# ddlau/modular_rl

Measured on AMD Instinct MI355X. Metric: env-steps/sec + TRPO-iters/sec, 4096 envs×1024 steps, 1/2/4/8 MI355X, higher is better.
Workload: dtype fp32

## Files before the change

### modular_rl_amd/csrc/fvp_split_role.h

```cpp
#pragma once
#include "../../include/mrl_hip.h"
#include "bf16_frag.h"
#include "mlp_device.h"
#include "rows_epilogue.h"

namespace mrl {

__host__ __device__ constexpr int split_fw(const BDims& b) { return b.fwd_words - b.fa0; }
__host__ __device__ constexpr int split_fwd_words(const BDims& b) { return b.fa0 + 3 * split_fw(b); }

__device__ inline float bf16_part(float v, int p) {
  const __bf16 a = (__bf16)v;
  if (p == 0) return (float)a;
  const float r = v - (float)a;
  const __bf16 c = (__bf16)r;
  if (p == 1) return (float)c;
  return r - (float)c;
}

__device__ inline int split_image_items(const BDims& b) { return b.fa0 + split_fw(b); }

__device__ inline void split_image_item(const MlpDims& d, const BDims& b, const float* th, float* image, int u) {
  if (u < b.fa0) {
    int idx;
    if (u < b.fb1) idx = d.fb0 + (u - b.fb0);
    else if (u < b.hv) idx = d.fb1 + (u - b.fb1);
    else if (u < b.hb) idx = d.hv + (u - b.hv);
    else idx = d.hb + (u - b.hb);
    image[u] = image_value(d, th, idx);
    return;
  }
  const int FW = split_fw(b);
  const int wp = u;
  int seg, rel;
  if (wp < b.fa1) { seg = 0; rel = wp - b.fa0; }
  else { seg = 1; rel = wp - b.fa1; }
  const int frag = rel >> 2, q = rel & 3;
  const float lo = bimage_elem(d, b, th, seg, frag, 2 * q), hi = bimage_elem(d, b, th, seg, frag, 2 * q + 1);
#pragma unroll
  for (int part = 0; part < 3; ++part) {
    const __bf16 l = (__bf16)bf16_part(lo, part), h = (__bf16)bf16_part(hi, part);
    image[u + part * FW] =
        __uint_as_float((uint32_t)__builtin_bit_cast(uint16_t, l) | ((uint32_t)__builtin_bit_cast(uint16_t, h) << 16));
  }
}

__device__ inline void split8v(const float* v, bf16x8* out) {
#pragma unroll
  for (int j = 0; j < 8; j += 2) {
    bf16x2 a, c, e;
    split2(f32x2{v[j], v[j + 1]}, a, c, e);
    out[0][j] = a[0];
    out[0][j + 1] = a[1];
    out[1][j] = c[0];
    out[1][j + 1] = c[1];
    out[2][j] = e[0];
    out[2][j + 1] = e[1];
  }
}
__device__ inline void split8(const f32x16& t, int sp, bf16x8* out) {
  float v[8];
#pragma unroll
  for (int j = 0; j < 8; ++j) v[j] = t[8 * sp + j];
  split8v(v, out);
}

__device__ inline void mfma_split(const float* img, int seg, int PS, int f, int lane, const bf16x8* x, f32x16& acc) {
  const bf16x8 w0 = frag_at(img, seg, f, lane), w1 = frag_at(img, seg + PS, f, lane);
  const bf16x8 w2 = frag_at(img, seg + 2 * PS, f, lane);
  acc = MFMA32B(w2, x[0], acc);
  acc = MFMA32B(w0, x[2], acc);
  acc = MFMA32B(w1, x[1], acc);
  acc = MFMA32B(w1, x[0], acc);
  acc = MFMA32B(w0, x[1], acc);
  acc = MFMA32B(w0, x[0], acc);
}

#define FVP_SPLIT_FENCE() __builtin_amdgcn_sched_barrier(0)

template <int SH>
__device__ inline void split_shape(RowsArgs& a, BDims& b) {
  if constexpr (SH != 0) {
    constexpr StaticShape S = STATIC_SHAPES[SH];
    a.d = static_dims(SH);
    a.A = S.A;
    a.head = S.head;
    a.n_obs = S.O;
    a.gh = S.head == MRL_HEAD_GAUSS ? 2 * S.A : S.A;
    a.ept = nullptr;
    b = bf16_dims(S.O, S.A);
  }
}

struct JvpSplitRole {
  RowsArgs a;
  BDims b;
  const float* img;
  const float* imt;
  MlpDims dd;
  int lane, h, PS;
  bool need_z;
  float xv[MAX_KS0B][8];
  f32x16 h1[2];

  __device__ __forceinline__ void init(const RowsArgs& a_, const BDims& b_, const float* img_, const float* imt_,
                                       int lane_) {
    a = a_;
    b = b_;
    img = img_;
    imt = imt_;
    dd = head_dims(a.d, b);
    lane = lane_;
    h = lane >> 5;
    PS = split_fw(b);
    need_z = a.head != MRL_HEAD_GAUSS;
  }
  __device__ __forceinline__ void load_xh1(int64_t t, float (&x)[MAX_KS0B][8], f32x16* hh) {
    const int64_t r = t * 32 + (lane & 31);
    XGlobalNB xl{a.x, a.ept, a.ts_limit, a.n_obs, r, r < a.n};
#pragma unroll
    for (int s0 = 0; s0 < MAX_KS0B; ++s0)
#pragma unroll
      for (int j = 0; j < 8; ++j) x[s0][j] = s0 < b.KS0B ? xl(16 * s0 + 8 * h + j) : 0.f;
    cache_load(a.cache + t * CACHE_TILE_FLOATS, lane, 0, hh[0]);
    cache_load(a.cache + t * CACHE_TILE_FLOATS, lane, 1, hh[1]);
  }
  __device__ __forceinline__ void prologue(int64_t tile) { load_xh1(tile, xv, h1); }
  template <bool PF = true, class Sink>
  __device__ __forceinline__ void tile(int64_t tile, int64_t tn, Sink&& sink) {
    const int64_t row = tile * 32 + (lane & 31);
    const bool valid = row < a.n;
    const float* ct = a.cache + tile * CACHE_TILE_FLOATS;
    f32x16 h2[2];
    if constexpr (PF) {
      cache_load(ct, lane, 2, h2[0]);
      cache_load(ct, lane, 3, h2[1]);
      __builtin_amdgcn_sched_barrier(0);
    }
    float xn[MAX_KS0B][8];
    f32x16 h1n[2];
    if constexpr (PF) load_xh1(tn, xn, h1n);
    else load_xh1(tile, xv, h1);
    __builtin_amdgcn_sched_barrier(0);
    f32x16 dh[2];
    dh[0] = load_bias16(imt, b.fb0, 0, h);
    dh[1] = load_bias16(imt, b.fb0, 1, h);
#pragma unroll
    for (int s0 = 0; s0 < MAX_KS0B; ++s0) {
      if (s0 < b.KS0B) {
        bf16x8 xs[3];
        split8v(xv[s0], xs);
        mfma_split(imt, b.fa0, PS, 0 * b.KS0B + s0, lane, xs, dh[0]);
        mfma_split(imt, b.fa0, PS, 1 * b.KS0B + s0, lane, xs, dh[1]);
      }
    }
    mul_dtanh16(dh[0], h1[0]);
    mul_dtanh16(dh[1], h1[1]);
    float z[MAX_OUT], dz[MAX_OUT], dzt[MAX_OUT];
#pragma unroll
    for (int o = 0; o < MAX_OUT; ++o) z[o] = dz[o] = dzt[o] = 0.f;
    f32x16 da2[2] = {load_bias16(imt, b.fb1, 0, h), load_bias16(imt, b.fb1, 1, h)};
#pragma unroll
    for (int s = 0; s < 4; ++s) {
      bf16x8 ps[3];
      split8(dh[s >> 1], s & 1, ps);
      mfma_split(img, b.fa1, PS, 0 * 4 + s, lane, ps, da2[0]);
      mfma_split(img, b.fa1, PS, 1 * 4 + s, lane, ps, da2[1]);
    }
    FVP_SPLIT_FENCE();
    if constexpr (!PF) {
      cache_load(ct, lane, 2, h2[0]);
      cache_load(ct, lane, 3, h2[1]);
      __builtin_amdgcn_sched_barrier(0);
    }
#pragma unroll
    for (int s = 0; s < 4; ++s) {
      bf16x8 ps[3];
      split8(h1[s >> 1], s & 1, ps);
      mfma_split(imt, b.fa1, PS, 0 * 4 + s, lane, ps, da2[0]);
      mfma_split(imt, b.fa1, PS, 1 * 4 + s, lane, ps, da2[1]);
    }
    FVP_SPLIT_FENCE();
#pragma unroll
    for (int mo = 0; mo < 2; ++mo) {
      f32x16& da = da2[mo];
      mul_dtanh16(da, h2[mo]);
      if (need_z) head_partial_mt(img, dd, h2[mo], mo, h, z);
      head_partial_mt(img, dd, da, mo, h, dz);
      head_partial_mt(imt, dd, h2[mo], mo, h, dzt);
      FVP_SPLIT_FENCE();
    }
    if (need_z) head_finish(img, dd, z);
#pragma unroll
    for (int o = 0; o < MAX_OUT; ++o) dz[o] += dzt[o];
    head_finish(imt, dd, dz);
    sink(valid, row, z, dz);
    if constexpr (PF) {
#pragma unroll
      for (int s0 = 0; s0 < MAX_KS0B; ++s0)
#pragma unroll
        for (int j = 0; j < 8; ++j) xv[s0][j] = xn[s0][j];
      h1[0] = h1n[0];
      h1[1] = h1n[1];
    }
  }
};

template <int EPI, bool LDSHEAD = false>
__device__ __forceinline__ void split_rows_tile(const RowsArgs& a, const BDims& b, const float* img, const MlpDims& dd,
                                                int lane, int64_t tile, bool store, const float (&ls)[MAX_OUT],
                                                const float (&sd)[MAX_OUT], const float (&dls)[MAX_OUT],
                                                double& acc0, double& acc1, double& acc2, const RowsArgs& ae,
                                                int64_t erow) {
  const int h = lane >> 5, PS = split_fw(b);
  const int64_t row = tile * 32 + (lane & 31);
  const bool valid = row < a.n;
  XGlobalNB xl{a.x, a.ept, a.ts_limit, a.n_obs, row, valid};
  float* ct = store ? a.cache + tile * CACHE_TILE_FLOATS : nullptr;
  f32x16 h1[2] = {load_bias16(img, b.fb0, 0, h), load_bias16(img, b.fb0, 1, h)};
#pragma unroll
  for (int s0 = 0; s0 < MAX_KS0B; ++s0) {
    if (s0 < b.KS0B) {
      float xv[8];
#pragma unroll
      for (int j = 0; j < 8; ++j) xv[j] = xl(16 * s0 + 8 * h + j);
      bf16x8 xs[3];
      split8v(xv, xs);
      mfma_split(img, b.fa0, PS, 0 * b.KS0B + s0, lane, xs, h1[0]);
      mfma_split(img, b.fa0, PS, 1 * b.KS0B + s0, lane, xs, h1[1]);
    }
  }
  tanh16(h1[0]);
  tanh16(h1[1]);
  if (store) {
    cache_store(ct, lane, 0, h1[0]);
    cache_store(ct, lane, 1, h1[1]);
  }
  f32x16 a2[2] = {load_bias16(img, b.fb1, 0, h), load_bias16(img, b.fb1, 1, h)};
#pragma unroll
  for (int s = 0; s < 4; ++s) {
    bf16x8 ps[3];
    split8(h1[s >> 1], s & 1, ps);
    mfma_split(img, b.fa1, PS, 0 * 4 + s, lane, ps, a2[0]);
    mfma_split(img, b.fa1, PS, 1 * 4 + s, lane, ps, a2[1]);
  }
  FVP_SPLIT_FENCE();
  float z[MAX_OUT], dz[MAX_OUT];
#pragma unroll
  for (int o = 0; o < MAX_OUT; ++o) z[o] = dz[o] = 0.f;
#pragma unroll
  for (int mo = 0; mo < 2; ++mo) {
    tanh16(a2[mo]);
    if (store) cache_store(ct, lane, 2 + mo, a2[mo]);
    head_partial_mt(img, dd, a2[mo], mo, h, z);
  }
  head_finish(img, dd, z);
  if constexpr (EPI == MRL_EPI_PROB)
    if (a.feat != nullptr && valid) write_feature_row(a, row, h, xl);
  if (valid && h == 0) row_epilogue<EPI, MAX_OUT, LDSHEAD>(ae, erow, z, dz, ls, sd, dls, acc0, acc1, acc2);
}

}
```

### modular_rl_amd/csrc/mlp_device.h

```cpp
#pragma once
#include "mlp_layout.h"

#define WAVE_LDS_ORDER() asm volatile("" ::: "memory")

namespace mrl {

__device__ inline f32x16 zero16() {
  f32x16 z;
#pragma unroll
  for (int i = 0; i < 16; ++i) z[i] = 0.f;
  return z;
}

__device__ inline float4 ld4(const float* p) { return *reinterpret_cast<const float4*>(p); }
__device__ inline float f4get(const float4& v, int q) { return q == 0 ? v.x : (q == 1 ? v.y : (q == 2 ? v.z : v.w)); }

__device__ inline f32x16 load_bias16(const float* lds, int off, int mo, int h) {
  const float* p = lds + off + (mo * 2 + h) * 16;
  const float4 a = ld4(p), b = ld4(p + 4), c = ld4(p + 8), e = ld4(p + 12);
  f32x16 r;
  r[0] = a.x; r[1] = a.y; r[2] = a.z; r[3] = a.w;
  r[4] = b.x; r[5] = b.y; r[6] = b.z; r[7] = b.w;
  r[8] = c.x; r[9] = c.y; r[10] = c.z; r[11] = c.w;
  r[12] = e.x; r[13] = e.y; r[14] = e.z; r[15] = e.w;
  return r;
}

__device__ inline float4 frag4(const float* lds, int seg, int KSp, int mo, int s4, int lane) {
  return reinterpret_cast<const float4*>(lds + seg)[(mo * (KSp / 4) + s4) * 64 + lane];
}

struct XGlobal {
  const float* x;
  const int32_t* ept;
  double ts_limit;
  int n_obs;
  int64_t row;
  bool valid;
  __device__ inline float operator()(int k) const {
    const int64_t r = valid ? row : 0;
    float v = 0.f;
    if (k < n_obs) v = x[r * n_obs + k];
    else if (ept != nullptr && k == n_obs) v = (float)((double)ept[r] / ts_limit);
    return valid ? v : 0.f;
  }
};

struct XGlobalNB {
  const float* x;
  const int32_t* ept;
  double ts_limit;
  int n_obs;
  int64_t row;
  bool valid;
  __device__ inline float operator()(int k) const {
    const int64_t r = valid ? row : 0;
    float f = (valid && k < n_obs) ? 1.f : 0.f;
    asm volatile("" : "+v"(f));
    float v = x[r * n_obs + (k < n_obs ? k : n_obs - 1)] * f;
    if (ept != nullptr && k == n_obs) v = valid ? (float)((double)ept[r] / ts_limit) : 0.f;
    return v;
  }
};

template <class XL>
__device__ inline void layer0(const float* lds, const MlpDims& d, const XL& xl, int lane, f32x16* acc) {
  const int h = lane >> 5;
  for (int s4 = 0; s4 < d.KS0p / 4; ++s4) {
    const float4 w0 = frag4(lds, d.fa0, d.KS0p, 0, s4, lane);
    const float4 w1 = frag4(lds, d.fa0, d.KS0p, 1, s4, lane);
    const float b0 = xl(8 * s4 + 0 + h), b1 = xl(8 * s4 + 2 + h);
    const float b2 = xl(8 * s4 + 4 + h), b3 = xl(8 * s4 + 6 + h);
    acc[0] = MFMA32(w0.x, b0, acc[0]);
    acc[1] = MFMA32(w1.x, b0, acc[1]);
    acc[0] = MFMA32(w0.y, b1, acc[0]);
    acc[1] = MFMA32(w1.y, b1, acc[1]);
    acc[0] = MFMA32(w0.z, b2, acc[0]);
    acc[1] = MFMA32(w1.z, b2, acc[1]);
    acc[0] = MFMA32(w0.w, b3, acc[0]);
    acc[1] = MFMA32(w1.w, b3, acc[1]);
  }
}

template <int MO>
__device__ inline void chain(const float* lds, int seg, const f32x16* src, int lane, f32x16* acc) {
#pragma unroll
  for (int s4 = 0; s4 < 8; ++s4) {
#pragma unroll
    for (int mo = 0; mo < MO; ++mo) {
      const float4 w = frag4(lds, seg, 32, mo, s4, lane);
      const int s = 4 * s4;
      acc[mo] = MFMA32(w.x, src[(s + 0) >> 4][(s + 0) & 15], acc[mo]);
      acc[mo] = MFMA32(w.y, src[(s + 1) >> 4][(s + 1) & 15], acc[mo]);
      acc[mo] = MFMA32(w.z, src[(s + 2) >> 4][(s + 2) & 15], acc[mo]);
      acc[mo] = MFMA32(w.w, src[(s + 3) >> 4][(s + 3) & 15], acc[mo]);
    }
  }
}

__device__ inline float tanh_fast(float x) {
  const float ax = fabsf(x);
  const float x2 = x * x;
  float q = fmaf(x2, -0.0539682545f, 0.133333340f);
  q = fmaf(x2, q, -0.333333343f);
  q = fmaf(x2, q, 1.f);
  const float p = x * q;
  const float e = __expf(2.f * ax);
  const float t = fmaf(-2.f, __builtin_amdgcn_rcpf(e + 1.f), 1.f);
  const float r = copysignf(t, x);
  return ax < 0.125f ? p : r;
}

typedef float f32x2 __attribute__((ext_vector_type(2)));
__device__ inline f32x2 tanh_fast2(f32x2 x) {
  const f32x2 ax = __builtin_elementwise_abs(x);
  const f32x2 x2 = x * x;
  f32x2 q = __builtin_elementwise_fma(x2, (f32x2)(-0.0539682545f), (f32x2)(0.133333340f));
  q = __builtin_elementwise_fma(x2, q, (f32x2)(-0.333333343f));
  q = __builtin_elementwise_fma(x2, q, (f32x2)(1.f));
  const f32x2 p = x * q;
  const f32x2 y = (ax + ax) * (f32x2)(__uint_as_float(0x3fb8aa3bu));
  f32x2 e;
  e.x = __builtin_amdgcn_exp2f(y.x);
  e.y = __builtin_amdgcn_exp2f(y.y);
  const f32x2 d = e + (f32x2)(1.f);
  f32x2 r;
  r.x = __builtin_amdgcn_rcpf(d.x);
  r.y = __builtin_amdgcn_rcpf(d.y);
  const f32x2 t = __builtin_elementwise_fma((f32x2)(-2.f), r, (f32x2)(1.f));
  f32x2 o;
  o.x = ax.x < 0.125f ? p.x : copysignf(t.x, x.x);
  o.y = ax.y < 0.125f ? p.y : copysignf(t.y, x.y);
  return o;
}

typedef __bf16 bf16x2 __attribute__((ext_vector_type(2)));
__device__ inline void split2(f32x2 v, bf16x2& a, bf16x2& c, bf16x2& e) {
  a = __builtin_convertvector(v, bf16x2);
  const f32x2 r = v - __builtin_convertvector(a, f32x2);
  c = __builtin_convertvector(r, bf16x2);
  e = __builtin_convertvector(r - __builtin_convertvector(c, f32x2), bf16x2);
}
__device__ inline void split4(const f32x4& v, bf16x4* p) {
  bf16x2 a0, c0, e0, a1, c1, e1;
  split2(f32x2{v[0], v[1]}, a0, c0, e0);
  split2(f32x2{v[2], v[3]}, a1, c1, e1);
  p[0] = __builtin_shufflevector(a0, a1, 0, 1, 2, 3);
  p[1] = __builtin_shufflevector(c0, c1, 0, 1, 2, 3);
  p[2] = __builtin_shufflevector(e0, e1, 0, 1, 2, 3);
}
__device__ inline bf16x8 cat4(const bf16x4& lo, const bf16x4& hi) {
  return __builtin_shufflevector(lo, hi, 0, 1, 2, 3, 4, 5, 6, 7);
}
typedef __bf16 bf16x16 __attribute__((ext_vector_type(16)));
__device__ inline bf16x16 split4w(const f32x4& v) {
  bf16x2 a0, c0, e0, a1, c1, e1;
  split2(f32x2{v[0], v[1]}, a0, c0, e0);
  split2(f32x2{v[2], v[3]}, a1, c1, e1);
  const bf16x4 p0 = __builtin_shufflevector(a0, a1, 0, 1, 2, 3);
  const bf16x4 p1 = __builtin_shufflevector(c0, c1, 0, 1, 2, 3);
  const bf16x4 p2 = __builtin_shufflevector(e0, e1, 0, 1, 2, 3);
  return __builtin_shufflevector(cat4(p0, p1), cat4(p2, p0), 0, 1, 2, 3, 4, 5, 6, 7, 8, 9, 10, 11, 12, 13, 14,
                                 15);
}
__device__ inline bf16x8 W0(const bf16x16& w) { return __builtin_shufflevector(w, w, 0, 1, 2, 3, 4, 5, 6, 7); }
__device__ inline bf16x8 W8(const bf16x16& w) { return __builtin_shufflevector(w, w, 8, 9, 10, 11, 12, 13, 14, 15); }

__device__ inline float dtanh(float h) { return fmaf(-h, h, 1.f); }
__device__ inline void mul_dtanh16(f32x16& t, const f32x16& h) {
#pragma unroll
  for (int r = 0; r < 16; r += 2) {
    const f32x2 hh = f32x2{h[r], h[r + 1]};
    const f32x2 d = __builtin_elementwise_fma(-hh, hh, (f32x2)(1.f));
    const f32x2 tt = f32x2{t[r], t[r + 1]} * d;
    t[r] = tt.x;
    t[r + 1] = tt.y;
  }
}

__device__ inline void tanh16(f32x16& a) {
#pragma unroll
  for (int r = 0; r < 16; r += 2) {
    const f32x2 t = tanh_fast2(f32x2{a[r], a[r + 1]});
    a[r] = t.x;
    a[r + 1] = t.y;
  }
}

__device__ inline void head_partial(const float* lds, const MlpDims& d, const f32x16* src, int h, float* z) {
  const float* w = lds + d.hv + h * (MAX_OUT * 32);
#pragma unroll
  for (int o = 0; o < MAX_OUT; ++o) {
    if (o < d.A) {
      float acc = 0.f;
#pragma unroll
      for (int q = 0; q < 8; ++q) {
        const float4 wv = ld4(w + o * 32 + 4 * q);
        const int mt = q >> 2, r0 = 4 * (q & 3);
        acc = fmaf(wv.x, src[mt][r0], acc);
        acc = fmaf(wv.y, src[mt][r0 + 1], acc);
        acc = fmaf(wv.z, src[mt][r0 + 2], acc);
        acc = fmaf(wv.w, src[mt][r0 + 3], acc);
      }
      z[o] += acc;
    }
  }
}

__device__ inline float xor32_add(float x) {
  const auto p = __builtin_amdgcn_permlane32_swap(__float_as_uint(x), __float_as_uint(x), false, false);
  return __uint_as_float(p[0]) + __uint_as_float(p[1]);
}
__device__ inline float xor16_add(float x) {
  const auto p = __builtin_amdgcn_permlane16_swap(__float_as_uint(x), __float_as_uint(x), false, false);
  return __uint_as_float(p[0]) + __uint_as_float(p[1]);
}
template <int CTRL>
__device__ inline float dpp_f(float x) {
  return __int_as_float(__builtin_amdgcn_mov_dpp(__float_as_int(x), CTRL, 0xF, 0xF, false));
}
__device__ inline float half_sum(float x) {
  x = xor16_add(x);
  x += dpp_f<0x128>(x);
  x += dpp_f<0x124>(x);
  x += dpp_f<0x4E>(x);
  x += dpp_f<0xB1>(x);
  return x;
}

__device__ inline void head_finish(const float* lds, const MlpDims& d, float* z) {
#pragma unroll
  for (int o = 0; o < MAX_OUT; ++o)
    if (o < d.A) z[o] = xor32_add(z[o]) + lds[d.hb + o];
}

__device__ inline void head_partial_mt(const float* lds, const MlpDims& d, const f32x16& src, int mt, int h,
                                       float* z) {
  const float* w = lds + d.hv + h * (MAX_OUT * 32) + mt * 16;
#pragma unroll
  for (int o = 0; o < MAX_OUT; ++o) {
    if (o < d.A) {
      float acc = 0.f;
#pragma unroll
      for (int q = 0; q < 4; ++q) {
        const float4 wv = ld4(w + o * 32 + 4 * q);
        acc = fmaf(wv.x, src[4 * q], acc);
        acc = fmaf(wv.y, src[4 * q + 1], acc);
        acc = fmaf(wv.z, src[4 * q + 2], acc);
        acc = fmaf(wv.w, src[4 * q + 3], acc);
      }
      z[o] += acc;
    }
  }
}

__device__ inline void chain1(const float* lds, int seg, int mo, const f32x16* src, int lane, f32x16& acc) {
#pragma unroll
  for (int s4 = 0; s4 < 8; ++s4) {
    const float4 w = frag4(lds, seg, 32, mo, s4, lane);
    const int s = 4 * s4;
    acc = MFMA32(w.x, src[(s + 0) >> 4][(s + 0) & 15], acc);
    acc = MFMA32(w.y, src[(s + 1) >> 4][(s + 1) & 15], acc);
    acc = MFMA32(w.z, src[(s + 2) >> 4][(s + 2) & 15], acc);
    acc = MFMA32(w.w, src[(s + 3) >> 4][(s + 3) & 15], acc);
  }
}

constexpr int CACHE_TILE_FLOATS = 64 * 64;
__device__ inline void cache_store(float* tile, int lane, int slot, const f32x16& v) {
#pragma unroll
  for (int q = 0; q < 4; ++q)
    reinterpret_cast<float4*>(tile)[(slot * 4 + q) * 64 + lane] =
        make_float4(v[4 * q], v[4 * q + 1], v[4 * q + 2], v[4 * q + 3]);
}
__device__ inline void cache_load(const float* tile, int lane, int slot, f32x16& v) {
#pragma unroll
  for (int q = 0; q < 4; ++q) {
    const float4 x = reinterpret_cast<const float4*>(tile)[(slot * 4 + q) * 64 + lane];
    v[4 * q] = x.x;
    v[4 * q + 1] = x.y;
    v[4 * q + 2] = x.z;
    v[4 * q + 3] = x.w;
  }
}

template <class XL>
__device__ inline void forward_head_lowreg(const float* lds, const MlpDims& d, const XL& xl, int lane, float* z,
                                           float* cache = nullptr) {
  const int h = lane >> 5;
  f32x16 h1[2];
  h1[0] = load_bias16(lds, d.fb0, 0, h);
  h1[1] = load_bias16(lds, d.fb0, 1, h);
  layer0(lds, d, xl, lane, h1);
  tanh16(h1[0]);
  tanh16(h1[1]);
  if (cache != nullptr) {
    cache_store(cache, lane, 0, h1[0]);
    cache_store(cache, lane, 1, h1[1]);
  }
#pragma unroll
  for (int o = 0; o < MAX_OUT; ++o) z[o] = 0.f;
#pragma unroll
  for (int mo = 0; mo < 2; ++mo) {
    f32x16 a = load_bias16(lds, d.fb1, mo, h);
    chain1(lds, d.fa1, mo, h1, lane, a);
    __builtin_amdgcn_sched_barrier(0);
    tanh16(a);
    if (cache != nullptr) cache_store(cache, lane, 2 + mo, a);
    head_partial_mt(lds, d, a, mo, h, z);
    __builtin_amdgcn_sched_barrier(0);
  }
  head_finish(lds, d, z);
}

template <class XL>
__device__ inline void jvp_head_cached(const float* lds, const float* ldt, const MlpDims& d, const XL& xl, int lane,
                                       const float* cache, float* z, float* dz, bool need_z = true) {
  const int h = lane >> 5;
  f32x16 h1[2], dh1[2];
  cache_load(cache, lane, 0, h1[0]);
  cache_load(cache, lane, 1, h1[1]);
  dh1[0] = load_bias16(ldt, d.fb0, 0, h);
  dh1[1] = load_bias16(ldt, d.fb0, 1, h);
  layer0(ldt, d, xl, lane, dh1);
#pragma unroll
  for (int m = 0; m < 2; ++m) mul_dtanh16(dh1[m], h1[m]);
  float dzt[MAX_OUT];
#pragma unroll
  for (int o = 0; o < MAX_OUT; ++o) {
    z[o] = 0.f;
    dz[o] = 0.f;
    dzt[o] = 0.f;
  }
#pragma unroll
  for (int mo = 0; mo < 2; ++mo) {
    f32x16 a;
    cache_load(cache, lane, 2 + mo, a);
    f32x16 da = load_bias16(ldt, d.fb1, mo, h);
    chain1(lds, d.fa1, mo, dh1, lane, da);
    __builtin_amdgcn_sched_barrier(0);
    chain1(ldt, d.fa1, mo, h1, lane, da);
    __builtin_amdgcn_sched_barrier(0);
    mul_dtanh16(da, a);
    if (need_z) head_partial_mt(lds, d, a, mo, h, z);
    head_partial_mt(lds, d, da, mo, h, dz);
    head_partial_mt(ldt, d, a, mo, h, dzt);
  }
  if (need_z) head_finish(lds, d, z);
#pragma unroll
  for (int o = 0; o < MAX_OUT; ++o) dz[o] += dzt[o];
  head_finish(ldt, d, dz);
}

template <class XL>
__device__ inline void forward_jvp_head_lowreg(const float* lds, const float* ldt, const MlpDims& d, const XL& xl,
                                               int lane, float* z, float* dz) {
  const int h = lane >> 5;
  f32x16 h1[2], dh1[2];
  h1[0] = load_bias16(lds, d.fb0, 0, h);
  h1[1] = load_bias16(lds, d.fb0, 1, h);
  layer0(lds, d, xl, lane, h1);
  dh1[0] = load_bias16(ldt, d.fb0, 0, h);
  dh1[1] = load_bias16(ldt, d.fb0, 1, h);
// ... 182 lines not shown
```

### modular_rl_amd/csrc/mlp_fisher.hip

```cpp
#include <math.h>

#include <type_traits>

#include "fvp_split_role.h"
#include "vjp16_device.h"

namespace mrl {

constexpr int MBOX_GH = 2 * MAX_OUT;
constexpr int HYB_W2_FLOATS = 2 * 4 * 64, HYB_WBS_FRAGS = 2 * 4 * 3 * 64;
constexpr size_t hyb_static_lds(int nslot) {
  return (size_t)HYB_W2_FLOATS * 4 + (size_t)HYB_VJP_WAVES * VJP16_H1_FLOATS * 4 + (size_t)HYB_WBS_FRAGS * 16 +
         (size_t)nslot * 4 * 32 * MBOX_GH * 4;
}

__device__ inline f32x4 ldv4(const f32x4* p) { return *p; }
__device__ inline float ldv1(const float* p) { return *p; }

struct FisherFusedIn {
  RowsArgs ra;
  BDims rb;
  const float* img_s;
  const float* imt_s;
};

template <int SH, int PROD = 0>
__global__ __launch_bounds__(64 * HYB_WAVES, 1) void mlp_fisher_hyb_kernel(VjpArgs a, const float* __restrict__ img,
                                                                         const int32_t* __restrict__ skip,
                                                                         FisherFusedIn fz) {
  constexpr int MT0 = 1;
  __shared__ __attribute__((aligned(16))) float lds[HYB_W2_FLOATS];
  __shared__ __attribute__((aligned(16))) float sH[HYB_VJP_WAVES * VJP16_H1_FLOATS];
  __shared__ __attribute__((aligned(16))) bf16x8 wbs[HYB_WBS_FRAGS];
  constexpr int LAG = PROD == 1 ? 2 : 1, NSLOT = LAG + 1;
  __shared__ __attribute__((aligned(16))) float mbox[NSLOT * 4 * 32 * MBOX_GH];
  static_assert(sizeof(lds) + sizeof(sH) + sizeof(wbs) + sizeof(mbox) == hyb_static_lds(NSLOT), "hyb_static_lds");
  extern __shared__ __attribute__((aligned(16))) float ldsx[];
  if (skip != nullptr && *skip != 0) return;
  const MlpDims& d = a.d;
  for (int i = threadIdx.x; i < HYB_W2_FLOATS / 4; i += 64 * HYB_WAVES)
    reinterpret_cast<float4*>(lds)[i] = reinterpret_cast<const float4*>(img + d.ba1 + 2 * 32 * 64)[i];
  const int WS = split_fwd_words(fz.rb);
  for (int i = threadIdx.x; i < WS / 4; i += 64 * HYB_WAVES) {
    reinterpret_cast<float4*>(ldsx)[i] = reinterpret_cast<const float4*>(fz.img_s)[i];
    if constexpr (PROD == 0) reinterpret_cast<float4*>(ldsx + WS)[i] = reinterpret_cast<const float4*>(fz.imt_s)[i];
  }
  const int lane = threadIdx.x & 63, c = lane & 15, g = lane >> 4;
  const int wave = __builtin_amdgcn_readfirstlane(threadIdx.x >> 6);
  const int A = d.A, gh = a.gh;
  const int KS2 = (A + 3) >> 2;
  const float* w2l = lds + 4 * c + g;
  auto w2frag = [&](int nt, int ks) { return w2l[((nt >> 1) * 64 + 32 * ks + 16 * (nt & 1)) * 4]; };
  __syncthreads();
  const float* w1l = img + d.ba1 + (32 * (g & 1) + c) * 4;
  auto w1frag = [&](int nt, int mt) {
    const int s4 = 4 * (mt >> 1) + 2 * (mt & 1) + (g >> 1);
    return ld4(w1l + (((nt >> 1) * 8 + s4) * 64 + 16 * (nt & 1)) * 4);
  };
  const int offT = ((c >> 3) * 64 + 32 * ((c >> 2) & 1) + 4 * g) * 4 + (c & 3);
  const int offR = ((g >> 1) * 64 + 32 * (g & 1) + c) * 4;
  {
    static_assert(HYB_WAVES >= 8, "one (s, nt) per wave of the first eight");
    if (wave < 8) {
      const int s = wave >> 2, nt = wave & 3;
      const float4 u = w1frag(nt, 2 * s), v = w1frag(nt, 2 * s + 1);
      bf16x4 pu[3], pv[3];
      split4(f32x4{u.x, u.y, u.z, u.w}, pu);
      split4(f32x4{v.x, v.y, v.z, v.w}, pv);
#pragma unroll
      for (int p = 0; p < 3; ++p) wbs[((s * 4 + nt) * 3 + p) * 64 + lane] = cat4(pu[p], pv[p]);
    }
    __syncthreads();
  }
  const int64_t nt32 = (a.n + 31) / 32, stride32 = (int64_t)gridDim.x * 4;
  const int64_t rounds = (nt32 + stride32 - 1) / stride32 + LAG;
  auto fused_barrier = []() {
    asm volatile("s_waitcnt lgkmcnt(0)" ::: "memory");
    __builtin_amdgcn_s_barrier();
    asm volatile("" ::: "memory");
  };
  if constexpr (PROD == 1) {
    if (wave < 4) {
      RowsArgs ra = fz.ra;
      BDims rb = fz.rb;
      split_shape<SH>(ra, rb);
      const MlpDims dd = head_dims(ra.d, rb);
      float ls[MAX_OUT], sd[MAX_OUT], dls[MAX_OUT];
#pragma unroll
      for (int j = 0; j < MAX_OUT; ++j) {
        ls[j] = (ra.logstd != nullptr && j < ra.A) ? ra.logstd[j] : 0.f;
        sd[j] = expf(ls[j]);
        dls[j] = 0.f;
      }
      const int A = ra.A, actw = ra.head == MRL_HEAD_SOFTMAX ? 1 : A, opw = ra.head == MRL_HEAD_SOFTMAX ? A : 2 * A;
      double acc0 = 0.0, acc1 = 0.0, acc2 = 0.0;
      int64_t T = (int64_t)blockIdx.x * 4 + wave;
      for (int64_t r = 0; r < rounds; ++r) {
        if (r + LAG < rounds && T < nt32) {
          float* mb = mbox + ((r % NSLOT) * 4 + wave) * 32 * MBOX_GH;
          const int64_t row0 = T * 32;
          RowsArgs ae = ra;
          ae.adv = ra.adv + row0;
          ae.act = ra.head == MRL_HEAD_SOFTMAX ? (const void*)(reinterpret_cast<const int32_t*>(ra.act) + row0)
                                               : (const void*)(reinterpret_cast<const float*>(ra.act) + row0 * actw);
          ae.oldprob = ra.oldprob + row0 * opw;
          ae.ghead = mb;
          ae.gh = MBOX_GH;
          if ((lane >> 5) == 0 && row0 + (lane & 31) >= ra.n)
            for (int j = 0; j < MBOX_GH; ++j) mb[(lane & 31) * MBOX_GH + j] = 0.f;
          split_rows_tile<MRL_EPI_SURRGRAD, true>(ra, rb, ldsx, dd, lane, T, true, ls, sd, dls, acc0, acc1, acc2, ae,
                                            lane & 31);
          T += stride32;
        }
        asm volatile("s_waitcnt vmcnt(0)" ::: "memory");
        fused_barrier();
      }
      acc0 = wave_sum(acc0);
      acc1 = wave_sum(acc1);
      acc2 = wave_sum(acc2);
      if (lane == 0) {
        double* p = ra.partial + ((int64_t)blockIdx.x * 4 + wave) * 4;
        p[0] = acc0;
        p[1] = acc1;
        p[2] = acc2;
        p[3] = 0.0;
      }
      return;
    }
  } else {
    if (wave < 4) {
      RowsArgs ra = fz.ra;
      BDims rb = fz.rb;
      split_shape<SH>(ra, rb);
      JvpSplitRole role;
      role.init(ra, rb, ldsx, ldsx + WS, lane);
      float sd[MAX_OUT], dls[MAX_OUT];
#pragma unroll
      for (int j = 0; j < MAX_OUT; ++j) {
        sd[j] = expf((ra.logstd != nullptr && j < ra.A) ? ra.logstd[j] : 0.f);
        dls[j] = (ra.dlogstd != nullptr && j < ra.A) ? ra.dlogstd[j] : 0.f;
      }
      int64_t T = (int64_t)blockIdx.x * 4 + wave;
      for (int64_t r = 0; r < rounds; ++r) {
        if (r + 1 < rounds && T < nt32) {
          const int64_t tn = T + stride32 < nt32 ? T + stride32 : T;
          float* mb = mbox + ((r & 1) * 4 + wave) * 32 * MBOX_GH + (lane & 31) * MBOX_GH;
          role.template tile<false>(T, tn, [&](bool valid, int64_t, const float (&z)[MAX_OUT],
                                                const float (&dz)[MAX_OUT]) {
            if ((lane >> 5) == 0) {
              float gg[MAX_OUT], gl[MAX_OUT];
              fvp_metric_row<MAX_OUT>(ra, z, dz, sd, dls, gg, gl);
#pragma unroll
              for (int j = 0; j < MAX_OUT; ++j)
                if (j < ra.A) {
                  mb[j] = valid ? gg[j] : 0.f;
                  if (ra.head == MRL_HEAD_GAUSS) mb[ra.A + j] = valid ? gl[j] : 0.f;
                }
            }
          });
          T += stride32;
        }
        fused_barrier();
      }
      return;
    }
  }

  auto vjp_role = [&](auto role_b) {
  constexpr bool RB = decltype(role_b)::value, RA = !RB;
  f32x4 gW1[4][4], gW2[4], gW0[MT0][4];
  f32x4 zero4 = f32x4{0.f, 0.f, 0.f, 0.f};
#pragma unroll
  for (int m = 0; m < 4; ++m) {
    gW2[m] = zero4;
#pragma unroll
    for (int n = 0; n < 4; ++n) gW1[m][n] = zero4;
#pragma unroll
    for (int m0 = 0; m0 < MT0; ++m0) gW0[m0][m] = zero4;
  }
  float pb1[4] = {0.f, 0.f, 0.f, 0.f}, pG = 0.f;

  const int64_t last = a.n - 1;
  float gq[2], GB[4], xA[MT0][4], xN[MT0][4];
  f32x4 h2R[4], h2T[4], h1T[4];
  auto load_h2 = [&](int64_t t) {
    const float* ct = a.cache + (t >> 1) * CACHE_TILE_FLOATS + 16 * (int)(t & 1) * 4;
    if constexpr (RB) {
#pragma unroll
      for (int nt = 0; nt < 4; ++nt)
        h2R[nt] = ldv4(reinterpret_cast<const f32x4*>(ct + (2 + (nt >> 1)) * 1024 + 512 * (nt & 1) + offR));
    } else {
#pragma unroll
      for (int nt = 0; nt < 4; ++nt)
#pragma unroll
        for (int r = 0; r < 4; ++r) h2T[nt][r] = ldv1(ct + (2 + (nt >> 1)) * 1024 + 512 * (nt & 1) + 4 * r + offT);
    }
  };
  const float* mbt = mbox;
  auto load_g_mbox = [&](int64_t t) {
    const float* m = mbt + 16 * (int)(t & 1) * MBOX_GH;
#pragma unroll
    for (int ks = 0; ks < 2; ++ks) {
      const int o = 4 * ks + g;
      gq[ks] = m[c * MBOX_GH + (o < gh ? o : gh - 1)];
    }
    if constexpr (RA) {
#pragma unroll
      for (int r = 0; r < 4; ++r) GB[r] = m[(4 * g + r) * MBOX_GH + (c < gh ? c : gh - 1)];
    }
  };
  auto mask_g = [&](int64_t t) {
    const int64_t row0 = t * 16;
#pragma unroll
    for (int ks = 0; ks < 2; ++ks) gq[ks] *= opaque((row0 + c < a.n && 4 * ks + g < A && ks < KS2) ? 1.f : 0.f);
    if constexpr (RA) {
#pragma unroll
      for (int r = 0; r < 4; ++r) GB[r] *= opaque((row0 + 4 * g + r < a.n && c < gh) ? 1.f : 0.f);
    }
  };
  auto take_x = [&]() {
    if constexpr (RA) return;
#pragma unroll
    for (int r = 0; r < 4; ++r) {
#pragma unroll
      for (int m0 = 0; m0 < MT0; ++m0) xA[m0][r] = xN[m0][r];
    }
  };
  auto load_x = [&](int64_t t) {
    if constexpr (RA) return;
    const int64_t row0 = t * 16;
#pragma unroll
    for (int r = 0; r < 4; ++r) {
      const int64_t rr = row0 + 4 * g + r, rc = rr < last ? rr : last;
#pragma unroll
      for (int m0 = 0; m0 < MT0; ++m0) {
        const int col = 16 * m0 + c;
        xN[m0][r] = ldv1(a.x + rc * a.n_obs + (col < a.n_obs ? col : a.n_obs - 1));
      }
    }
  };
  float* const h1s = sH + (wave - 4) * VJP16_H1_FLOATS;
  auto dma_h1 = [&](int64_t t) {
    const float* ct = a.cache + (t >> 1) * CACHE_TILE_FLOATS + 16 * (int)(t & 1) * 4;
    const int jj = lane & 15;
#pragma unroll
    for (int i = 0; i < 4; ++i) {
      const int run = 4 * i + (lane >> 4), sq = run >> 1, hh = run & 1, k = 2 * (sq & 1) + hh;
      const int j = 4 * (jj >> 2) + ((jj - k) & 3);
      glds16(ct + (sq * 64 + 32 * hh + j) * 4, h1s + i * 256);
    }
  };
  int offH[4];
#pragma unroll
  for (int r = 0; r < 4; ++r)
    offH[r] = ((c >> 3) * 2 + ((c >> 2) & 1)) * 64 + 16 * g + 4 * ((r + (c >> 2)) & 3) + (c & 3);
  auto read_h1 = [&](int nt) {
    const float* p = h1s + (nt >> 1) * 512 + (nt & 1) * 256;
    h1T[nt] = f32x4{p[offH[0]], p[offH[1]], p[offH[2]], p[offH[3]]};
  };
  auto mask_x = [&]() {
    if constexpr (RA) return;
#pragma unroll
    for (int r = 0; r < 4; ++r)
#pragma unroll
      for (int m0 = 0; m0 < MT0; ++m0) {
        const int col = 16 * m0 + c;
        float xv = xA[m0][r] * opaque(col < a.n_obs ? 1.f : 0.f) + (col == d.O ? 1.f : 0.f);
        xA[m0][r] = xv;
      }
  };
  auto vjp_tile = [&](int64_t t, int64_t tn) {
    load_g_mbox(t);
    mask_g(t);
    f32x4 ga2[4];
#pragma unroll
    for (int nt = 0; nt < 4; ++nt) {
      const float w = w2frag(nt, 0);
      ga2[nt] = RB ? MFMA16(w, gq[0], zero4) : MFMA16(gq[0], w, zero4);
    }
    if (KS2 > 1) {
#pragma unroll
      for (int nt = 0; nt < 4; ++nt) {
        const float w = w2frag(nt, 1);
        ga2[nt] = RB ? MFMA16(w, gq[1], ga2[nt]) : MFMA16(gq[1], w, ga2[nt]);
      }
    }
    if constexpr (RA) {
#pragma unroll
      for (int r = 0; r < 4; ++r)
#pragma unroll
        for (int nt = 0; nt < 4; ++nt) gW2[nt] = MFMA16(h2T[nt][r], GB[r], gW2[nt]);
#pragma unroll
      for (int r = 0; r < 4; ++r) pG += GB[r];
    }
#pragma unroll
    for (int nt = 0; nt < 4; ++nt)
#pragma unroll
      for (int r = 0; r < 4; ++r) ga2[nt][r] *= dtanh(RB ? h2R[nt][r] : h2T[nt][r]);
    if constexpr (RA) {
#pragma unroll
      for (int nt = 0; nt < 4; ++nt) pb1[nt] += (ga2[nt][0] + ga2[nt][1]) + (ga2[nt][2] + ga2[nt][3]);
    }
    __builtin_amdgcn_sched_barrier(0);
    f32x4 g1T[4] = {zero4, zero4, zero4, zero4};
    asm volatile("s_waitcnt vmcnt(0)" ::: "memory");
    if constexpr (RB) {
#pragma unroll
      for (int nt = 0; nt < 4; ++nt) read_h1(nt);
    }
    {
      if constexpr (RA) {
        bf16x16 gw[4];
#pragma unroll
        for (int nt = 0; nt < 4; ++nt) gw[nt] = split4w(ga2[nt]);
#pragma unroll
        for (int mt = 0; mt < 4; ++mt) {
          read_h1(mt);
          const bf16x16 hw = split4w(h1T[mt]);
#pragma unroll
          for (int nt = 0; nt < 4; ++nt) {
            gW1[mt][nt] = MFMAB16(W8(hw), W0(gw[nt]), gW1[mt][nt]);
            gW1[mt][nt] = MFMAB16(W0(hw), W8(gw[nt]), gW1[mt][nt]);
            gW1[mt][nt] = MFMAB16(W0(hw), W0(gw[nt]), gW1[mt][nt]);
          }
        }
      }
      __builtin_amdgcn_sched_barrier(0);
      load_h2(tn);
      load_x(tn);
      asm volatile("s_waitcnt lgkmcnt(0)" ::: "memory");
      dma_h1(tn);
      __builtin_amdgcn_sched_barrier(0);
      if constexpr (RB) {
#pragma unroll
      for (int s = 0; s < 2; ++s) {
        bf16x4 pa[3], pb[3];
        split4(ga2[2 * s], pa);
        split4(ga2[2 * s + 1], pb);
        const bf16x8 A0 = cat4(pa[0], pb[0]), A1 = cat4(pa[1], pb[1]), A2 = cat4(pa[2], pb[2]);
#pragma unroll
        for (int nt = 0; nt < 4; ++nt) {
          const bf16x8* w = wbs + (s * 4 + nt) * 3 * 64 + lane;
          const bf16x8 B0 = w[0], B1 = w[64], B2 = w[128];
          g1T[nt] = MFMAB16(A2, B0, g1T[nt]);
          g1T[nt] = MFMAB16(A0, B2, g1T[nt]);
          g1T[nt] = MFMAB16(A1, B1, g1T[nt]);
          g1T[nt] = MFMAB16(A1, B0, g1T[nt]);
          g1T[nt] = MFMAB16(A0, B1, g1T[nt]);
          g1T[nt] = MFMAB16(A0, B0, g1T[nt]);
        }
      }
      }
    }
    if constexpr (RB) {
#pragma unroll
      for (int nt = 0; nt < 4; ++nt)
#pragma unroll
        for (int r = 0; r < 4; ++r) g1T[nt][r] *= dtanh(h1T[nt][r]);
      mask_x();
#pragma unroll
      for (int r = 0; r < 4; ++r)
#pragma unroll
        for (int m0 = 0; m0 < MT0; ++m0)
#pragma unroll
          for (int nt = 0; nt < 4; ++nt) gW0[m0][nt] = MFMA16(xA[m0][r], g1T[nt][r], gW0[m0][nt]);
      take_x();
    }
  };
  {
    const int vw = (wave - 4) & 3;
    int64_t T = (int64_t)blockIdx.x * 4 + vw;
    for (int64_t r = 0; r < LAG; ++r) {
      if (r == LAG - 1 && T < nt32) {
        load_h2(2 * T);
        load_x(2 * T);
        dma_h1(2 * T);
        take_x();
      }
      fused_barrier();
    }
    for (int64_t r = LAG; r < rounds; ++r) {
      if (T < nt32) {
        mbt = mbox + (((r - LAG) % NSLOT) * 4 + vw) * 32 * MBOX_GH;
        const int64_t Tn = T + stride32 < nt32 ? T + stride32 : T;
#pragma unroll 1
        for (int hf = 0; hf < 2; ++hf) vjp_tile(2 * T + hf, hf ? 2 * Tn : 2 * T + 1);
        T += stride32;
      }
      fused_barrier();
    }
  }

  asm volatile("s_waitcnt vmcnt(0)" ::: "memory");
  float* out = a.slab + ((int64_t)blockIdx.x * 4 + ((wave - 4) & 3)) * d.P;
  if constexpr (RB) {
#pragma unroll
    for (int m0 = 0; m0 < MT0; ++m0)
#pragma unroll
      for (int n = 0; n < 4; ++n)
#pragma unroll
        for (int r = 0; r < 4; ++r) {
          const int i = 16 * m0 + 4 * g + r;
          if (i < d.O) out[d.tW0 + i * HID + 16 * n + c] = gW0[m0][n][r];
          else if (i == d.O) out[d.tb0 + 16 * n + c] = gW0[m0][n][r];
        }
    return;
  }
#pragma unroll
  for (int nt = 0; nt < 4; ++nt) pb1[nt] = xor32_add(xor16_add(pb1[nt]));
  pG = xor32_add(xor16_add(pG));
#pragma unroll
  for (int m = 0; m < 4; ++m)
#pragma unroll
    for (int n = 0; n < 4; ++n)
// ... 123 lines not shown
```

### modular_rl_amd/csrc/mlp_split.hip

```cpp
#include <math.h>
#include <stdlib.h>

#include "../../include/mrl_hip.h"
#include "bf16_frag.h"
#include "mlp_device.h"
#include "rows_epilogue.h"
#include "fvp_split_role.h"
#include "mlp_host.h"

namespace mrl {

__global__ void mlp_pack_split_kernel(MlpDims d, BDims b, const float* __restrict__ th, float* __restrict__ image,
                                      int items, const int32_t* __restrict__ skip) {
  if (skip != nullptr && *skip != 0) return;
  const int u = blockIdx.x * blockDim.x + threadIdx.x;
  if (u < items) split_image_item(d, b, th, image, u);
}

#ifndef MRL_SPLIT_ROWS_WAVES
#define MRL_SPLIT_ROWS_WAVES 4
#endif
constexpr int SPLIT_ROWS_WAVES = MRL_SPLIT_ROWS_WAVES;
constexpr int SPLIT_ROWS_BLOCK = 64 * SPLIT_ROWS_WAVES;

#ifndef MRL_SPLIT_FVP_OCC
#define MRL_SPLIT_FVP_OCC 2
#endif
template <int SH>
__global__ __launch_bounds__(SPLIT_ROWS_BLOCK, (4 * MRL_SPLIT_FVP_OCC / SPLIT_ROWS_WAVES > 0
                                                 ? 4 * MRL_SPLIT_FVP_OCC / SPLIT_ROWS_WAVES : 1))
    void mlp_fvp_split_kernel(RowsArgs a, BDims b, const float* __restrict__ img_g, const float* __restrict__ imt_g,
                              const int32_t* __restrict__ skip) {
  split_shape<SH>(a, b);
  extern __shared__ __attribute__((aligned(16))) float lds[];
  if (skip != nullptr && *skip != 0) return;
  const int W = split_fwd_words(b);
  for (int i = threadIdx.x; i < W / 4; i += SPLIT_ROWS_BLOCK) {
    reinterpret_cast<float4*>(lds)[i] = reinterpret_cast<const float4*>(img_g)[i];
    reinterpret_cast<float4*>(lds + W)[i] = reinterpret_cast<const float4*>(imt_g)[i];
  }
  __syncthreads();
  const int lane = threadIdx.x & 63;
  const int wave = __builtin_amdgcn_readfirstlane(threadIdx.x >> 6);
  JvpSplitRole role;
  role.init(a, b, lds, lds + W, lane);
  const int A = a.A;
  float ls[MAX_OUT], sd[MAX_OUT], dls[MAX_OUT];
#pragma unroll
  for (int j = 0; j < MAX_OUT; ++j) {
    ls[j] = (a.logstd != nullptr && j < A) ? a.logstd[j] : 0.f;
    sd[j] = expf(ls[j]);
    dls[j] = (a.dlogstd != nullptr && j < A) ? a.dlogstd[j] : 0.f;
  }
  double acc0 = 0.0, acc1 = 0.0, acc2 = 0.0;
  const int64_t ntiles = (a.n + 31) / 32;
  const int64_t stride = (int64_t)gridDim.x * SPLIT_ROWS_WAVES;
  const int h = lane >> 5;
  int64_t tile = (int64_t)blockIdx.x * SPLIT_ROWS_WAVES + wave;
  if (tile < ntiles) role.prologue(tile);
  for (; tile < ntiles; tile += stride) {
    const int64_t tn = tile + stride < ntiles ? tile + stride : tile;
    role.tile(tile, tn, [&](bool valid, int64_t row, const float (&z)[MAX_OUT], const float (&dz)[MAX_OUT]) {
      if (valid && h == 0) row_epilogue<MRL_EPI_FVP, MAX_OUT>(a, row, z, dz, ls, sd, dls, acc0, acc1, acc2);
    });
  }
  (void)acc0;
  (void)acc1;
  (void)acc2;
}


template <int SH>
__device__ inline void split_rows_shape(RowsArgs& a, BDims& b) {
  if constexpr ((SH & ~SH_TIME) != 0) {
    constexpr int B = SH & ~SH_TIME;
    constexpr StaticShape S = STATIC_SHAPES[B];
    a.d = static_dims(B);
    a.A = S.A;
    a.head = S.head;
    a.n_obs = (SH & SH_TIME) ? S.O - 1 : S.O;
    a.gh = S.head == MRL_HEAD_GAUSS ? 2 * S.A : S.A;
    if constexpr (!(SH & SH_TIME)) a.ept = nullptr;
    b = bf16_dims(S.O, S.A);
  }
}

template <int EPI, int SH>
__global__ __launch_bounds__(SPLIT_ROWS_BLOCK, 2) void mlp_rows_split_kernel(RowsArgs a, BDims b,
                                                                            const float* __restrict__ img_g,
                                                                            const int32_t* __restrict__ skip) {
  split_rows_shape<SH>(a, b);
  extern __shared__ __attribute__((aligned(16))) float lds[];
  if (skip != nullptr && *skip != 0) return;
  const int W = split_fwd_words(b);
  for (int i = threadIdx.x; i < W / 4; i += SPLIT_ROWS_BLOCK)
    reinterpret_cast<float4*>(lds)[i] = reinterpret_cast<const float4*>(img_g)[i];
  __syncthreads();
  const float* img = lds;
  const MlpDims dd = head_dims(a.d, b);
  const int lane = threadIdx.x & 63;
  const int wave = __builtin_amdgcn_readfirstlane(threadIdx.x >> 6);
  const int A = a.A;
  float ls[MAX_OUT], sd[MAX_OUT], dls[MAX_OUT];
#pragma unroll
  for (int j = 0; j < MAX_OUT; ++j) {
    ls[j] = (a.logstd != nullptr && j < A) ? a.logstd[j] : 0.f;
    sd[j] = expf(ls[j]);
    dls[j] = 0.f;
  }
  const bool store = a.cache != nullptr && a.cache_mode == MRL_CACHE_WRITE;
  double acc0 = 0.0, acc1 = 0.0, acc2 = 0.0;
  const int64_t ntiles = (a.n + 31) / 32;
  for (int64_t tile = (int64_t)blockIdx.x * SPLIT_ROWS_WAVES + wave; tile < ntiles;
       tile += (int64_t)gridDim.x * SPLIT_ROWS_WAVES) {
    const int64_t row = tile * 32 + (lane & 31);
    split_rows_tile<EPI>(a, b, img, dd, lane, tile, store, ls, sd, dls, acc0, acc1, acc2, a, row);
  }
  if (a.partial != nullptr) {
    acc0 = wave_sum(acc0);
    acc1 = wave_sum(acc1);
    acc2 = wave_sum(acc2);
    if (lane == 0) {
      double* p = a.partial + ((int64_t)blockIdx.x * SPLIT_ROWS_WAVES + wave) * 4;
      p[0] = acc0;
      p[1] = acc1;
      p[2] = acc2;
      p[3] = 0.0;
    }
  }
}

int launch_rows_split(int epi, int sh, const RowsArgs& a, const BDims& b, const float* image_s, int64_t blocks,
                      const int32_t* skip, void* stream) {
  const dim3 grid(blocks), blk(SPLIT_ROWS_BLOCK);
  const size_t shm = (size_t)split_fwd_words(b) * 4;
  hipStream_t s = (hipStream_t)stream;
#define MRL_RS(E, S) hipLaunchKernelGGL((mlp_rows_split_kernel<E, S>), grid, blk, shm, s, a, b, image_s, skip)
  switch (epi) {
    case MRL_EPI_PROB:
      if (sh == 1) MRL_RS(MRL_EPI_PROB, 1);
      else if (sh == 2) MRL_RS(MRL_EPI_PROB, 2);
      else if (sh == 3) MRL_RS(MRL_EPI_PROB, 3);
      else if (sh == 4) MRL_RS(MRL_EPI_PROB, 4);
      else if (sh == (3 | SH_TIME)) MRL_RS(MRL_EPI_PROB, 3 | SH_TIME);
      else if (sh == (4 | SH_TIME)) MRL_RS(MRL_EPI_PROB, 4 | SH_TIME);
      else MRL_RS(MRL_EPI_PROB, 0);
      break;
    case MRL_EPI_LOSSES:
      if (sh == 1) MRL_RS(MRL_EPI_LOSSES, 1);
      else if (sh == 2) MRL_RS(MRL_EPI_LOSSES, 2);
      else MRL_RS(MRL_EPI_LOSSES, 0);
      break;
    case MRL_EPI_SURRGRAD:
      if (sh == 1) MRL_RS(MRL_EPI_SURRGRAD, 1);
      else if (sh == 2) MRL_RS(MRL_EPI_SURRGRAD, 2);
      else MRL_RS(MRL_EPI_SURRGRAD, 0);
      break;
    case MRL_EPI_VFLOSS:
      if (sh == 3) MRL_RS(MRL_EPI_VFLOSS, 3);
      else if (sh == 4) MRL_RS(MRL_EPI_VFLOSS, 4);
      else MRL_RS(MRL_EPI_VFLOSS, 0);
      break;
    default:
      return fail(E_UNSUPPORTED, "mrl_mlp_rows_split: epilogue");
  }
#undef MRL_RS
  return hip_check(hipGetLastError(), "mrl_mlp_rows_split");
}

}

using namespace mrl;

static int64_t split_rows_blocks(int64_t n) {
  static const int64_t env_cap = [] {
    const char* e = getenv("MRL_SPLIT_BLOCKS");
    return (int64_t)(e ? atoi(e) : 0);
  }();
  const int64_t cap = env_cap > 0 ? env_cap : 2 * 256 * (4 * MRL_SPLIT_FVP_OCC / SPLIT_ROWS_WAVES > 0
                                                         ? 4 * MRL_SPLIT_FVP_OCC / SPLIT_ROWS_WAVES : 1);
  int64_t g = ceil_div(ceil_div(n, 32), SPLIT_ROWS_WAVES);
  if (g < 1) g = 1;
  return g > cap ? cap : g;
}

extern "C" {

int64_t mrl_mlp_image_words_split(const mrl_mlp_desc* d) {
  if (check_desc(d) != OK) return -1;
  return split_fwd_words(bf16_dims(d->n_in, d->n_out));
}

int mrl_mlp_pack_split(const mrl_mlp_desc* d, const float* theta, float* image, const int32_t* skip, void* stream) {
  int rc = check_desc(d);
  if (rc) return rc;
  if (!theta || !image) return fail(E_ARG, "null pointer");
  const MlpDims m = dims_of(d);
  const BDims b = bf16_dims(d->n_in, d->n_out);
  const int items = b.fa0 + split_fw(b);
  hipLaunchKernelGGL(mlp_pack_split_kernel, dim3((items + 255) / 256), dim3(256), 0, (hipStream_t)stream, m, b, theta,
                     image, items, skip);
  return hip_check(hipGetLastError(), "mrl_mlp_pack_split");
}

int mrl_mlp_fvp_split(const mrl_mlp_desc* d, const float* theta, const float* image, const float* tangent,
                      const float* image_t, const mrl_rows_io* io, const int32_t* skip, void* stream) {
  int rc = check_desc(d);
  if (rc) return rc;
  if (!io || !image || !image_t || !tangent || !io->x || !io->ghead) return fail(E_ARG, "null pointer");
  if (!io->act_cache || io->cache_mode != MRL_CACHE_READ)
    return fail(E_ARG, "mrl_mlp_fvp_split reads the f32 activation cache (MRL_CACHE_READ)");
  if (io->ep_t) return fail(E_ARG, "mrl_mlp_fvp_split: policy rows only (no time feature)");
  if (d->head == MRL_HEAD_LINEAR) return fail(E_ARG, "Fisher product of a value net");
  if (d->head == MRL_HEAD_GAUSS && !theta) return fail(E_ARG, "DiagGauss needs theta (logstd)");
  if (io->n <= 0) return OK;
  RowsArgs a{};
  a.d = dims_of(d);
  a.head = d->head;
  a.n_obs = d->n_in;
  a.gh = d->head == MRL_HEAD_GAUSS ? 2 * d->n_out : d->n_out;
  a.A = d->n_out;
  a.x = io->x;
  a.n = io->n;
  a.inv_ng = io->inv_n_global;
  a.ghead = io->ghead;
  a.logstd = (d->head == MRL_HEAD_GAUSS && theta) ? theta + a.d.tls : nullptr;
  a.dlogstd = (d->head == MRL_HEAD_GAUSS && tangent) ? tangent + a.d.tls : nullptr;
  a.cache = io->act_cache;
  a.cache_mode = MRL_CACHE_READ;
  const BDims b = bf16_dims(d->n_in, d->n_out);
  const size_t shm = (size_t)split_fwd_words(b) * 4 * 2;
  const dim3 grid(split_rows_blocks(io->n)), blk(SPLIT_ROWS_BLOCK);
  hipStream_t s = (hipStream_t)stream;
  switch (static_shape_of(d, false)) {
    case 1: hipLaunchKernelGGL((mlp_fvp_split_kernel<1>), grid, blk, shm, s, a, b, image, image_t, skip); break;
    case 2: hipLaunchKernelGGL((mlp_fvp_split_kernel<2>), grid, blk, shm, s, a, b, image, image_t, skip); break;
    default: hipLaunchKernelGGL((mlp_fvp_split_kernel<0>), grid, blk, shm, s, a, b, image, image_t, skip); break;
  }
  return hip_check(hipGetLastError(), "mrl_mlp_fvp_split");
}

}
```

Measured before the change: 151.1 million.

## Prefetch next tile's observations in split rows kernels and raise occupancy

Adds a RowsTileIn register buffer so each wave loads the next tile's raw observation inputs (and episode time) before computing the current tile. This software pipelining is applied to the split rows kernel for static shapes and to the fisher surrogate-gradient path, so global load latency overlaps with MFMA work. The feature-row write is moved into the input loop so it reuses the already-loaded values, and launch bounds are raised from 2 to 3 blocks per CU. The extra prefetch registers plus the tighter register budget from the higher launch bound risk spills.

```diff
diff --git a/modular_rl_amd/csrc/fvp_split_role.h b/modular_rl_amd/csrc/fvp_split_role.h
--- a/modular_rl_amd/csrc/fvp_split_role.h
+++ b/modular_rl_amd/csrc/fvp_split_role.h
@@ -206,12 +206,28 @@
   }
 };
 
+struct RowsTileIn {
+  float x[MAX_KS0B][8];
+  int32_t t;
+  __device__ __forceinline__ void load(const RowsArgs& a, const BDims& b, int lane, int64_t tile) {
+    const int h = lane >> 5;
+    const int64_t row = tile * 32 + (lane & 31);
+    const bool valid = row < a.n;
+    XGlobalNB xl{a.x, a.ept, a.ts_limit, a.n_obs, row, valid};
+#pragma unroll
+    for (int s0 = 0; s0 < MAX_KS0B; ++s0)
+#pragma unroll
+      for (int j = 0; j < 8; ++j) x[s0][j] = s0 < b.KS0B ? xl.raw(16 * s0 + 8 * h + j) : 0.f;
+    t = xl.raw_t();
+  }
+};
+
 template <int EPI, bool LDSHEAD = false>
 __device__ __forceinline__ void split_rows_tile(const RowsArgs& a, const BDims& b, const float* img, const MlpDims& dd,
-                                                int lane, int64_t tile, bool store, const float (&ls)[MAX_OUT],
-                                                const float (&sd)[MAX_OUT], const float (&dls)[MAX_OUT],
-                                                double& acc0, double& acc1, double& acc2, const RowsArgs& ae,
-                                                int64_t erow) {
+                                                int lane, int64_t tile, bool store, const RowsTileIn& in,
+                                                const float (&ls)[MAX_OUT], const float (&sd)[MAX_OUT],
+                                                const float (&dls)[MAX_OUT], double& acc0, double& acc1, double& acc2,
+                                                const RowsArgs& ae, int64_t erow) {
   const int h = lane >> 5, PS = split_fw(b);
   const int64_t row = tile * 32 + (lane & 31);
   const bool valid = row < a.n;
@@ -223,7 +239,15 @@
     if (s0 < b.KS0B) {
       float xv[8];
 #pragma unroll
-      for (int j = 0; j < 8; ++j) xv[j] = xl(16 * s0 + 8 * h + j);
+      for (int j = 0; j < 8; ++j) xv[j] = xl.use(in.x[s0][j], in.t, 16 * s0 + 8 * h + j);
+      if constexpr (EPI == MRL_EPI_PROB) {
+        if (a.feat != nullptr && valid) {
+          float* f = a.feat + row * (a.n_obs + 1);
+#pragma unroll
+          for (int j = 0; j < 8; ++j)
+            if (16 * s0 + 8 * h + j <= a.n_obs) f[16 * s0 + 8 * h + j] = xv[j];
+        }
+      }
       bf16x8 xs[3];
       split8v(xv, xs);
       mfma_split(img, b.fa0, PS, 0 * b.KS0B + s0, lane, xs, h1[0]);
@@ -255,8 +279,6 @@
     head_partial_mt(img, dd, a2[mo], mo, h, z);
   }
   head_finish(img, dd, z);
-  if constexpr (EPI == MRL_EPI_PROB)
-    if (a.feat != nullptr && valid) write_feature_row(a, row, h, xl);
   if (valid && h == 0) row_epilogue<EPI, MAX_OUT, LDSHEAD>(ae, erow, z, dz, ls, sd, dls, acc0, acc1, acc2);
 }
 
diff --git a/modular_rl_amd/csrc/mlp_device.h b/modular_rl_amd/csrc/mlp_device.h
--- a/modular_rl_amd/csrc/mlp_device.h
+++ b/modular_rl_amd/csrc/mlp_device.h
@@ -59,6 +59,15 @@
     asm volatile("" : "+v"(f));
     float v = x[r * n_obs + (k < n_obs ? k : n_obs - 1)] * f;
     if (ept != nullptr && k == n_obs) v = valid ? (float)((double)ept[r] / ts_limit) : 0.f;
+    return v;
+  }
+  __device__ inline float raw(int k) const { return x[(valid ? row : 0) * n_obs + (k < n_obs ? k : n_obs - 1)]; }
+  __device__ inline int32_t raw_t() const { return ept != nullptr ? ept[valid ? row : 0] : 0; }
+  __device__ inline float use(float xr, int32_t t, int k) const {
+    float f = (valid && k < n_obs) ? 1.f : 0.f;
+    asm volatile("" : "+v"(f));
+    float v = xr * f;
+    if (ept != nullptr && k == n_obs) v = valid ? (float)((double)t / ts_limit) : 0.f;
     return v;
   }
 };
diff --git a/modular_rl_amd/csrc/mlp_fisher.hip b/modular_rl_amd/csrc/mlp_fisher.hip
--- a/modular_rl_amd/csrc/mlp_fisher.hip
+++ b/modular_rl_amd/csrc/mlp_fisher.hip
@@ -95,8 +95,12 @@
       const int A = ra.A, actw = ra.head == MRL_HEAD_SOFTMAX ? 1 : A, opw = ra.head == MRL_HEAD_SOFTMAX ? A : 2 * A;
       double acc0 = 0.0, acc1 = 0.0, acc2 = 0.0;
       int64_t T = (int64_t)blockIdx.x * 4 + wave;
+      RowsTileIn in, nx;
+      if (T < nt32) in.load(ra, rb, lane, T);
       for (int64_t r = 0; r < rounds; ++r) {
         if (r + LAG < rounds && T < nt32) {
+          nx.load(ra, rb, lane, T + stride32 < nt32 ? T + stride32 : T);
+          __builtin_amdgcn_sched_barrier(0);
           float* mb = mbox + ((r % NSLOT) * 4 + wave) * 32 * MBOX_GH;
           const int64_t row0 = T * 32;
           RowsArgs ae = ra;
@@ -108,8 +112,9 @@
           ae.gh = MBOX_GH;
           if ((lane >> 5) == 0 && row0 + (lane & 31) >= ra.n)
             for (int j = 0; j < MBOX_GH; ++j) mb[(lane & 31) * MBOX_GH + j] = 0.f;
-          split_rows_tile<MRL_EPI_SURRGRAD, true>(ra, rb, ldsx, dd, lane, T, true, ls, sd, dls, acc0, acc1, acc2, ae,
-                                            lane & 31);
+          split_rows_tile<MRL_EPI_SURRGRAD, true>(ra, rb, ldsx, dd, lane, T, true, in, ls, sd, dls, acc0, acc1, acc2,
+                                                  ae, lane & 31);
+          in = nx;
           T += stride32;
         }
         asm volatile("s_waitcnt vmcnt(0)" ::: "memory");
diff --git a/modular_rl_amd/csrc/mlp_split.hip b/modular_rl_amd/csrc/mlp_split.hip
--- a/modular_rl_amd/csrc/mlp_split.hip
+++ b/modular_rl_amd/csrc/mlp_split.hip
@@ -86,7 +86,7 @@
 }
 
 template <int EPI, int SH>
-__global__ __launch_bounds__(SPLIT_ROWS_BLOCK, 2) void mlp_rows_split_kernel(RowsArgs a, BDims b,
+__global__ __launch_bounds__(SPLIT_ROWS_BLOCK, 3) void mlp_rows_split_kernel(RowsArgs a, BDims b,
                                                                             const float* __restrict__ img_g,
                                                                             const int32_t* __restrict__ skip) {
   split_rows_shape<SH>(a, b);
@@ -111,10 +111,21 @@
   const bool store = a.cache != nullptr && a.cache_mode == MRL_CACHE_WRITE;
   double acc0 = 0.0, acc1 = 0.0, acc2 = 0.0;
   const int64_t ntiles = (a.n + 31) / 32;
-  for (int64_t tile = (int64_t)blockIdx.x * SPLIT_ROWS_WAVES + wave; tile < ntiles;
-       tile += (int64_t)gridDim.x * SPLIT_ROWS_WAVES) {
-    const int64_t row = tile * 32 + (lane & 31);
-    split_rows_tile<EPI>(a, b, img, dd, lane, tile, store, ls, sd, dls, acc0, acc1, acc2, a, row);
+  constexpr bool PF = (SH & ~SH_TIME) != 0;
+  const int64_t stride = (int64_t)gridDim.x * SPLIT_ROWS_WAVES;
+  int64_t tile = (int64_t)blockIdx.x * SPLIT_ROWS_WAVES + wave;
+  RowsTileIn in, nx;
+  if (PF && tile < ntiles) in.load(a, b, lane, tile);
+  for (; tile < ntiles; tile += stride) {
+    if constexpr (PF) {
+      nx.load(a, b, lane, tile + stride < ntiles ? tile + stride : tile);
+      __builtin_amdgcn_sched_barrier(0);
+    } else {
+      in.load(a, b, lane, tile);
+    }
+    split_rows_tile<EPI>(a, b, img, dd, lane, tile, store, in, ls, sd, dls, acc0, acc1, acc2, a,
+                         tile * 32 + (lane & 31));
+    if constexpr (PF) in = nx;
   }
   if (a.partial != nullptr) {
     acc0 = wave_sum(acc0);
```

After: 151.0 million. Within noise of the previous version (-0.0%).
